# daniabib/ComfyUI_ProPainter_Nodes

Measured on NVIDIA H100. Metric: inpainted frames/sec at 640x360, 80-frame subvideo, higher is better.
Workload: dtype f16

## Files before the change

### comfyui_propainter_nodes_b200/csrc/attention_tc.cu

```cuda
#include "attention.cuh"
#include "wgmma_ops.cuh"

namespace {

constexpr int D = 128, BQ = 128, BKEY = 64, NT = 256, WIN_TOK = 45, RING = 193;
constexpr uint32_t QPANEL = BQ * 128;
constexpr uint32_t KPANEL = BKEY * 128;
constexpr uint32_t QTILE = 2 * QPANEL;
constexpr uint32_t KTILE = 2 * KPANEL;
constexpr uint32_t PTILE = (BKEY / 64) * QPANEL;
constexpr uint32_t SM_Q = 0, SM_K = QTILE, SM_V = SM_K + 2 * KTILE, SM_P = SM_V + 2 * KTILE, SM_END = SM_P + PTILE;

__device__ __forceinline__ uint32_t tile_off(uint32_t panel, int row, int chunk) {
  return (uint32_t)(chunk >> 3) * panel + (uint32_t)row * 128 + (uint32_t)(((chunk & 7) ^ (row & 7)) << 4);
}

__global__ void attn_key_table(int* __restrict__ tab, const int* __restrict__ ring_idx, int nk_max, int kpf, int ntok,
                               int n_pool, int qkv_cs, int pool_cs, int parity) {
  const int win = blockIdx.x;
  const int* ring = ring_idx + win * RING;
  for (int j = threadIdx.x; j < nk_max; j += blockDim.x) {
    const int fi = j / kpf, w = j - fi * kpf;
    const int fr = parity + 2 * fi;
    unsigned e;
    if (w < RING) e = (unsigned)(((long long)fr * ntok + ring[w]) * qkv_cs / 8);
    else e = 0x80000000u | (unsigned)(((long long)fr * n_pool + (w - RING)) * pool_cs / 8);
    tab[(long long)win * nk_max + j] = (int)e;
  }
}

__global__ void __launch_bounds__(NT, 2) window_attention_tc(const PPAttnParams p) {
  using namespace ppx;
  extern __shared__ __align__(1024) uint8_t smem[];
  const uint32_t sbase = smem_u32(smem);

  const int win = blockIdx.y >> 2, head = blockIdx.y & 3, sw = blockIdx.z;
  if (p.win_flags[sw * p.n_win + win] == 0) return;
  const int t = p.sw_t[sw];
  const int frame_base = p.sw_frame_off[sw];
  const int nq = t * WIN_TOK;
  const int q0 = blockIdx.x * BQ;
  if (q0 >= nq) return;
  const int n_tind = (t - p.parity + 1) / 2;
  const int kpf = RING + p.n_pool;
  const int nk = n_tind * kpf;
  const int ntiles = (nk + BKEY - 1) / BKEY;
  const int tid = threadIdx.x;
  const int* ring = p.ring_idx + win * RING;
  const long long ntok = (long long)p.nh * p.nw;

  for (int i = tid; i < BQ * 16; i += NT) {
    const int r = i >> 4, ch = i & 15;
    const int qi = min(q0 + r, nq - 1);
    const int fr = frame_base + qi / WIN_TOK, pos = qi % WIN_TOK;
    const __half* src = p.q + ((long long)fr * ntok + ring[pos]) * p.qkv_cs + head * D + ch * 8;
    cp_async16(sbase + SM_Q + tile_off(QPANEL, r, ch), src, 16);
  }
  const int r0 = tid >> 4, ch = tid & 15;
  const long long fb = frame_base;
  const __half* kb = p.k + fb * ntok * p.qkv_cs + head * D + ch * 8;
  const __half* vb = p.v + fb * ntok * p.qkv_cs + head * D + ch * 8;
  const __half* pkb = p.pk + fb * p.n_pool * p.pool_cs + head * D + ch * 8;
  const __half* pvb = p.pv + fb * p.n_pool * p.pool_cs + head * D + ch * 8;
  const int* ktab = p.key_tab + (long long)win * p.key_tab_stride;
  const uint32_t kv_dst0 = sbase + tile_off(KPANEL, r0, ch);
  auto load_kv = [&](int tile, int stage) {
    const uint32_t dk = kv_dst0 + SM_K + stage * KTILE, dv = kv_dst0 + SM_V + stage * KTILE;
#pragma unroll
    for (int it = 0; it < BKEY / 16; ++it) {
      const int j = tile * BKEY + r0 + 16 * it;
      const __half* ks = kb; const __half* vs = vb;
      uint32_t nbytes = 0;
      if (j < nk) {
        nbytes = 16;
        const int e = __ldg(ktab + j);
        const long long off = (long long)(e & 0x7fffffff) * 8;
        ks = (e < 0 ? pkb : kb) + off;
        vs = (e < 0 ? pvb : vb) + off;
      }
      cp_async16(dk + it * 2048, ks, nbytes);
      cp_async16(dv + it * 2048, vs, nbytes);
    }
    cp_async_commit();
  };
  load_kv(0, 0);

  const int wg = tid >> 7, lane = tid & 31;
  const int rw = 16 * ((tid >> 5) & 3) + (lane >> 2), quad = lane & 3;
  const uint32_t q_rows = (uint32_t)wg * 64 * 128;
  float o[64];
  float m_used[2] = {0.f, 0.f}, m_run[2] = {-1e30f, -1e30f}, row_sum[2] = {0.f, 0.f};
#pragma unroll
  for (int i = 0; i < 64; ++i) o[i] = 0.f;
  for (int j = 0; j < ntiles; ++j) {
    const int stage = j & 1;
    cp_async_wait<0>();
    fence_proxy_async();
    __syncthreads();
    if (j + 1 < ntiles) load_kv(j + 1, stage ^ 1);
    float s[32];
    wgmma_fence();
#pragma unroll
    for (int ks = 0; ks < 8; ++ks) {
      const uint32_t sub = (uint32_t)(ks & 3) * 32;
      wgmma_f16<BKEY>(s, gmma_desc_sw128_kmajor(sbase + SM_Q + (uint32_t)(ks >> 2) * QPANEL + q_rows + sub),
                      gmma_desc_sw128_kmajor(sbase + SM_K + stage * KTILE + (uint32_t)(ks >> 2) * KPANEL + sub), ks != 0 ? 1u : 0u);
    }
    wgmma_commit();
    wgmma_wait<0>();
    wgmma_fence_acc(s);

    const int kvalid = min(BKEY, nk - j * BKEY);
    float mx[2] = {-1e30f, -1e30f};
#pragma unroll
    for (int i = 0; i < 32; ++i) {
      if (8 * (i >> 2) + 2 * quad + (i & 1) >= kvalid) s[i] = -1e30f;
      mx[(i >> 1) & 1] = fmaxf(mx[(i >> 1) & 1], s[i]);
    }
    float f[2];
#pragma unroll
    for (int h = 0; h < 2; ++h) {
      mx[h] = fmaxf(mx[h], __shfl_xor_sync(0xffffffffu, mx[h], 1));
      mx[h] = fmaxf(mx[h], __shfl_xor_sync(0xffffffffu, mx[h], 2));
      const float m_tile = __half2float(__float2half_rn(fmaxf(mx[h] * p.scale_log2, -60000.f)));
      const float m_new = fmaxf(m_run[h], m_tile);
      f[h] = 1.f;
      if (j == 0) m_used[h] = m_new;
      else if (m_new > m_used[h] + 8.f) {
        f[h] = exp2f(m_used[h] - m_new);
        m_used[h] = m_new;
        row_sum[h] *= f[h];
      }
      m_run[h] = m_new;
    }
    if (f[0] != 1.f || f[1] != 1.f) {
#pragma unroll
      for (int i = 0; i < 64; ++i) o[i] *= f[(i >> 1) & 1];
    }
#pragma unroll
    for (int i = 0; i < 32; i += 2) {
      const int h = (i >> 1) & 1;
      const float a = exp2f(fmaf(s[i], p.scale_log2, -m_used[h]));
      const float b = exp2f(fmaf(s[i + 1], p.scale_log2, -m_used[h]));
      row_sum[h] += a + b;
      const int row = wg * 64 + rw + 8 * h;
      *reinterpret_cast<__half2*>(smem + SM_P + tile_off(QPANEL, row, i >> 2) + 4 * quad) = __floats2half2_rn(a, b);
    }
    fence_proxy_async();
    named_bar(1 + wg, 128);
    wgmma_fence();
#pragma unroll
    for (int ks = 0; ks < BKEY / 16; ++ks) {
      const uint64_t adesc = gmma_desc_sw128_kmajor(sbase + SM_P + q_rows + (uint32_t)ks * 32);
      const uint64_t bdesc = gmma_desc_sw128_mnmajor(sbase + SM_V + stage * KTILE + (uint32_t)ks * 2048, KPANEL);
      wgmma_f16<D, 1>(o, adesc, bdesc, 1u);
    }
    wgmma_commit();
    wgmma_wait<0>();
    wgmma_fence_acc(o);
  }

#pragma unroll
  for (int h = 0; h < 2; ++h) {
    row_sum[h] += __shfl_xor_sync(0xffffffffu, row_sum[h], 1);
    row_sum[h] += __shfl_xor_sync(0xffffffffu, row_sum[h], 2);
    const float inv = 1.f / row_sum[h];
    const int qi = q0 + wg * 64 + rw + 8 * h;
    if (qi >= nq) continue;
    const int fr = frame_base + qi / WIN_TOK, pos = qi % WIN_TOK;
    const int tok = ring[pos];
    const int ty = tok / p.nw, tx = tok - ty * p.nw;
    if (ty >= p.gh || tx >= p.gw) continue;
    __half* dst = p.out + (((long long)fr * p.gh + ty) * p.gw + tx) * p.out_cs + head * D + 2 * quad;
#pragma unroll
    for (int g = 0; g < D / 8; ++g)
      *reinterpret_cast<__half2*>(dst + 8 * g) = __floats2half2_rn(o[4 * g + 2 * h] * inv, o[4 * g + 2 * h + 1] * inv);
  }
}

}

int pp_launch_attention_tc(const PPAttnParams& p, int n_sliding, int t_max, cudaStream_t st) {
  const size_t smem = SM_END;
  static bool attr_set = false;
  if (!attr_set) {
    PP_CUDA_CHECK(cudaFuncSetAttribute(window_attention_tc, cudaFuncAttributeMaxDynamicSharedMemorySize, (int)smem));
    PP_CUDA_CHECK(cudaFuncSetAttribute(window_attention_tc, cudaFuncAttributePreferredSharedMemoryCarveout, 100));
    attr_set = true;
  }
  {
    const int kpf = RING + p.n_pool, nk_max = ((t_max - p.parity + 1) / 2) * kpf;
    PP_REQUIRE(p.key_tab != nullptr && p.key_tab_stride >= nk_max, "attention: key table scratch too small (%d < %d)",
               p.key_tab_stride, nk_max);
    attn_key_table<<<p.n_win, 256, 0, st>>>(const_cast<int*>(p.key_tab), p.ring_idx, p.key_tab_stride, kpf, p.nh * p.nw, p.n_pool,
                                           p.qkv_cs, p.pool_cs, p.parity);
    PP_CUDA_CHECK(cudaGetLastError());
  }
  dim3 grid(pp_ceil_div(t_max * WIN_TOK, BQ), p.n_win * 4, n_sliding);
  window_attention_tc<<<grid, NT, smem, st>>>(p);
  PP_CUDA_CHECK(cudaGetLastError());
  return PP_OK;
}
```

### comfyui_propainter_nodes_b200/csrc/wgmma_ops.cuh

```cuda
#pragma once
#include <stdint.h>

namespace ppx {

template <int N, int TB>
struct WgmmaF16;

template <int TB>
struct WgmmaF16<16, TB> {
  static __device__ __forceinline__ void run(float (&d)[8], uint64_t a, uint64_t b, uint32_t acc) {
    asm volatile(
        "{\n.reg .pred p;\nsetp.ne.b32 p, %10, 0;\n"
        "wgmma.mma_async.sync.aligned.m64n16k16.f32.f16.f16 {%0, %1, %2, %3, %4, %5, %6, %7}, %8, %9, p, 1, 1, 0, %11;\n}\n"
        : "+f"(d[0]), "+f"(d[1]), "+f"(d[2]), "+f"(d[3]), "+f"(d[4]), "+f"(d[5]), "+f"(d[6]), "+f"(d[7])
        : "l"(a), "l"(b), "r"(acc), "n"(TB)
        : "memory");
  }
};

template <int TB>
struct WgmmaF16<32, TB> {
  static __device__ __forceinline__ void run(float (&d)[16], uint64_t a, uint64_t b, uint32_t acc) {
    asm volatile(
        "{\n.reg .pred p;\nsetp.ne.b32 p, %18, 0;\n"
// ... 97 lines not shown
        : "+f"(d[0]), "+f"(d[1]), "+f"(d[2]), "+f"(d[3]), "+f"(d[4]), "+f"(d[5]), "+f"(d[6]), "+f"(d[7]), "+f"(d[8]), "+f"(d[9]), "+f"(d[10]), "+f"(d[11]), "+f"(d[12]), "+f"(d[13]), "+f"(d[14]), "+f"(d[15]), "+f"(d[16]), "+f"(d[17]), "+f"(d[18]), "+f"(d[19]), "+f"(d[20]), "+f"(d[21]), "+f"(d[22]), "+f"(d[23]), "+f"(d[24]), "+f"(d[25]), "+f"(d[26]), "+f"(d[27]), "+f"(d[28]), "+f"(d[29]), "+f"(d[30]), "+f"(d[31]), "+f"(d[32]), "+f"(d[33]), "+f"(d[34]), "+f"(d[35]), "+f"(d[36]), "+f"(d[37]), "+f"(d[38]), "+f"(d[39]), "+f"(d[40]), "+f"(d[41]), "+f"(d[42]), "+f"(d[43]), "+f"(d[44]), "+f"(d[45]), "+f"(d[46]), "+f"(d[47]), "+f"(d[48]), "+f"(d[49]), "+f"(d[50]), "+f"(d[51]), "+f"(d[52]), "+f"(d[53]), "+f"(d[54]), "+f"(d[55]), "+f"(d[56]), "+f"(d[57]), "+f"(d[58]), "+f"(d[59]), "+f"(d[60]), "+f"(d[61]), "+f"(d[62]), "+f"(d[63]), "+f"(d[64]), "+f"(d[65]), "+f"(d[66]), "+f"(d[67]), "+f"(d[68]), "+f"(d[69]), "+f"(d[70]), "+f"(d[71]), "+f"(d[72]), "+f"(d[73]), "+f"(d[74]), "+f"(d[75]), "+f"(d[76]), "+f"(d[77]), "+f"(d[78]), "+f"(d[79])
        : "l"(a), "l"(b), "r"(acc), "n"(TB)
        : "memory");
  }
};

template <int TB>
struct WgmmaF16<176, TB> {
  static __device__ __forceinline__ void run(float (&d)[88], uint64_t a, uint64_t b, uint32_t acc) {
    asm volatile(
        "{\n.reg .pred p;\nsetp.ne.b32 p, %90, 0;\n"
        "wgmma.mma_async.sync.aligned.m64n176k16.f32.f16.f16 {%0, %1, %2, %3, %4, %5, %6, %7, %8, %9, %10, %11, %12, %13, %14, %15, %16, %17, %18, %19, %20, %21, %22, %23, %24, %25, %26, %27, %28, %29, %30, %31, %32, %33, %34, %35, %36, %37, %38, %39, %40, %41, %42, %43, %44, %45, %46, %47, %48, %49, %50, %51, %52, %53, %54, %55, %56, %57, %58, %59, %60, %61, %62, %63, %64, %65, %66, %67, %68, %69, %70, %71, %72, %73, %74, %75, %76, %77, %78, %79, %80, %81, %82, %83, %84, %85, %86, %87}, %88, %89, p, 1, 1, 0, %91;\n}\n"
        : "+f"(d[0]), "+f"(d[1]), "+f"(d[2]), "+f"(d[3]), "+f"(d[4]), "+f"(d[5]), "+f"(d[6]), "+f"(d[7]), "+f"(d[8]), "+f"(d[9]), "+f"(d[10]), "+f"(d[11]), "+f"(d[12]), "+f"(d[13]), "+f"(d[14]), "+f"(d[15]), "+f"(d[16]), "+f"(d[17]), "+f"(d[18]), "+f"(d[19]), "+f"(d[20]), "+f"(d[21]), "+f"(d[22]), "+f"(d[23]), "+f"(d[24]), "+f"(d[25]), "+f"(d[26]), "+f"(d[27]), "+f"(d[28]), "+f"(d[29]), "+f"(d[30]), "+f"(d[31]), "+f"(d[32]), "+f"(d[33]), "+f"(d[34]), "+f"(d[35]), "+f"(d[36]), "+f"(d[37]), "+f"(d[38]), "+f"(d[39]), "+f"(d[40]), "+f"(d[41]), "+f"(d[42]), "+f"(d[43]), "+f"(d[44]), "+f"(d[45]), "+f"(d[46]), "+f"(d[47]), "+f"(d[48]), "+f"(d[49]), "+f"(d[50]), "+f"(d[51]), "+f"(d[52]), "+f"(d[53]), "+f"(d[54]), "+f"(d[55]), "+f"(d[56]), "+f"(d[57]), "+f"(d[58]), "+f"(d[59]), "+f"(d[60]), "+f"(d[61]), "+f"(d[62]), "+f"(d[63]), "+f"(d[64]), "+f"(d[65]), "+f"(d[66]), "+f"(d[67]), "+f"(d[68]), "+f"(d[69]), "+f"(d[70]), "+f"(d[71]), "+f"(d[72]), "+f"(d[73]), "+f"(d[74]), "+f"(d[75]), "+f"(d[76]), "+f"(d[77]), "+f"(d[78]), "+f"(d[79]), "+f"(d[80]), "+f"(d[81]), "+f"(d[82]), "+f"(d[83]), "+f"(d[84]), "+f"(d[85]), "+f"(d[86]), "+f"(d[87])
        : "l"(a), "l"(b), "r"(acc), "n"(TB)
        : "memory");
  }
};

template <int TB>
struct WgmmaF16<192, TB> {
  static __device__ __forceinline__ void run(float (&d)[96], uint64_t a, uint64_t b, uint32_t acc) {
    asm volatile(
        "{\n.reg .pred p;\nsetp.ne.b32 p, %98, 0;\n"
        "wgmma.mma_async.sync.aligned.m64n192k16.f32.f16.f16 {%0, %1, %2, %3, %4, %5, %6, %7, %8, %9, %10, %11, %12, %13, %14, %15, %16, %17, %18, %19, %20, %21, %22, %23, %24, %25, %26, %27, %28, %29, %30, %31, %32, %33, %34, %35, %36, %37, %38, %39, %40, %41, %42, %43, %44, %45, %46, %47, %48, %49, %50, %51, %52, %53, %54, %55, %56, %57, %58, %59, %60, %61, %62, %63, %64, %65, %66, %67, %68, %69, %70, %71, %72, %73, %74, %75, %76, %77, %78, %79, %80, %81, %82, %83, %84, %85, %86, %87, %88, %89, %90, %91, %92, %93, %94, %95}, %96, %97, p, 1, 1, 0, %99;\n}\n"
        : "+f"(d[0]), "+f"(d[1]), "+f"(d[2]), "+f"(d[3]), "+f"(d[4]), "+f"(d[5]), "+f"(d[6]), "+f"(d[7]), "+f"(d[8]), "+f"(d[9]), "+f"(d[10]), "+f"(d[11]), "+f"(d[12]), "+f"(d[13]), "+f"(d[14]), "+f"(d[15]), "+f"(d[16]), "+f"(d[17]), "+f"(d[18]), "+f"(d[19]), "+f"(d[20]), "+f"(d[21]), "+f"(d[22]), "+f"(d[23]), "+f"(d[24]), "+f"(d[25]), "+f"(d[26]), "+f"(d[27]), "+f"(d[28]), "+f"(d[29]), "+f"(d[30]), "+f"(d[31]), "+f"(d[32]), "+f"(d[33]), "+f"(d[34]), "+f"(d[35]), "+f"(d[36]), "+f"(d[37]), "+f"(d[38]), "+f"(d[39]), "+f"(d[40]), "+f"(d[41]), "+f"(d[42]), "+f"(d[43]), "+f"(d[44]), "+f"(d[45]), "+f"(d[46]), "+f"(d[47]), "+f"(d[48]), "+f"(d[49]), "+f"(d[50]), "+f"(d[51]), "+f"(d[52]), "+f"(d[53]), "+f"(d[54]), "+f"(d[55]), "+f"(d[56]), "+f"(d[57]), "+f"(d[58]), "+f"(d[59]), "+f"(d[60]), "+f"(d[61]), "+f"(d[62]), "+f"(d[63]), "+f"(d[64]), "+f"(d[65]), "+f"(d[66]), "+f"(d[67]), "+f"(d[68]), "+f"(d[69]), "+f"(d[70]), "+f"(d[71]), "+f"(d[72]), "+f"(d[73]), "+f"(d[74]), "+f"(d[75]), "+f"(d[76]), "+f"(d[77]), "+f"(d[78]), "+f"(d[79]), "+f"(d[80]), "+f"(d[81]), "+f"(d[82]), "+f"(d[83]), "+f"(d[84]), "+f"(d[85]), "+f"(d[86]), "+f"(d[87]), "+f"(d[88]), "+f"(d[89]), "+f"(d[90]), "+f"(d[91]), "+f"(d[92]), "+f"(d[93]), "+f"(d[94]), "+f"(d[95])
        : "l"(a), "l"(b), "r"(acc), "n"(TB)
        : "memory");
  }
};

template <int TB>
struct WgmmaF16<208, TB> {
  static __device__ __forceinline__ void run(float (&d)[104], uint64_t a, uint64_t b, uint32_t acc) {
    asm volatile(
        "{\n.reg .pred p;\nsetp.ne.b32 p, %106, 0;\n"
        "wgmma.mma_async.sync.aligned.m64n208k16.f32.f16.f16 {%0, %1, %2, %3, %4, %5, %6, %7, %8, %9, %10, %11, %12, %13, %14, %15, %16, %17, %18, %19, %20, %21, %22, %23, %24, %25, %26, %27, %28, %29, %30, %31, %32, %33, %34, %35, %36, %37, %38, %39, %40, %41, %42, %43, %44, %45, %46, %47, %48, %49, %50, %51, %52, %53, %54, %55, %56, %57, %58, %59, %60, %61, %62, %63, %64, %65, %66, %67, %68, %69, %70, %71, %72, %73, %74, %75, %76, %77, %78, %79, %80, %81, %82, %83, %84, %85, %86, %87, %88, %89, %90, %91, %92, %93, %94, %95, %96, %97, %98, %99, %100, %101, %102, %103}, %104, %105, p, 1, 1, 0, %107;\n}\n"
        : "+f"(d[0]), "+f"(d[1]), "+f"(d[2]), "+f"(d[3]), "+f"(d[4]), "+f"(d[5]), "+f"(d[6]), "+f"(d[7]), "+f"(d[8]), "+f"(d[9]), "+f"(d[10]), "+f"(d[11]), "+f"(d[12]), "+f"(d[13]), "+f"(d[14]), "+f"(d[15]), "+f"(d[16]), "+f"(d[17]), "+f"(d[18]), "+f"(d[19]), "+f"(d[20]), "+f"(d[21]), "+f"(d[22]), "+f"(d[23]), "+f"(d[24]), "+f"(d[25]), "+f"(d[26]), "+f"(d[27]), "+f"(d[28]), "+f"(d[29]), "+f"(d[30]), "+f"(d[31]), "+f"(d[32]), "+f"(d[33]), "+f"(d[34]), "+f"(d[35]), "+f"(d[36]), "+f"(d[37]), "+f"(d[38]), "+f"(d[39]), "+f"(d[40]), "+f"(d[41]), "+f"(d[42]), "+f"(d[43]), "+f"(d[44]), "+f"(d[45]), "+f"(d[46]), "+f"(d[47]), "+f"(d[48]), "+f"(d[49]), "+f"(d[50]), "+f"(d[51]), "+f"(d[52]), "+f"(d[53]), "+f"(d[54]), "+f"(d[55]), "+f"(d[56]), "+f"(d[57]), "+f"(d[58]), "+f"(d[59]), "+f"(d[60]), "+f"(d[61]), "+f"(d[62]), "+f"(d[63]), "+f"(d[64]), "+f"(d[65]), "+f"(d[66]), "+f"(d[67]), "+f"(d[68]), "+f"(d[69]), "+f"(d[70]), "+f"(d[71]), "+f"(d[72]), "+f"(d[73]), "+f"(d[74]), "+f"(d[75]), "+f"(d[76]), "+f"(d[77]), "+f"(d[78]), "+f"(d[79]), "+f"(d[80]), "+f"(d[81]), "+f"(d[82]), "+f"(d[83]), "+f"(d[84]), "+f"(d[85]), "+f"(d[86]), "+f"(d[87]), "+f"(d[88]), "+f"(d[89]), "+f"(d[90]), "+f"(d[91]), "+f"(d[92]), "+f"(d[93]), "+f"(d[94]), "+f"(d[95]), "+f"(d[96]), "+f"(d[97]), "+f"(d[98]), "+f"(d[99]), "+f"(d[100]), "+f"(d[101]), "+f"(d[102]), "+f"(d[103])
        : "l"(a), "l"(b), "r"(acc), "n"(TB)
        : "memory");
  }
};

template <int TB>
struct WgmmaF16<224, TB> {
  static __device__ __forceinline__ void run(float (&d)[112], uint64_t a, uint64_t b, uint32_t acc) {
    asm volatile(
        "{\n.reg .pred p;\nsetp.ne.b32 p, %114, 0;\n"
        "wgmma.mma_async.sync.aligned.m64n224k16.f32.f16.f16 {%0, %1, %2, %3, %4, %5, %6, %7, %8, %9, %10, %11, %12, %13, %14, %15, %16, %17, %18, %19, %20, %21, %22, %23, %24, %25, %26, %27, %28, %29, %30, %31, %32, %33, %34, %35, %36, %37, %38, %39, %40, %41, %42, %43, %44, %45, %46, %47, %48, %49, %50, %51, %52, %53, %54, %55, %56, %57, %58, %59, %60, %61, %62, %63, %64, %65, %66, %67, %68, %69, %70, %71, %72, %73, %74, %75, %76, %77, %78, %79, %80, %81, %82, %83, %84, %85, %86, %87, %88, %89, %90, %91, %92, %93, %94, %95, %96, %97, %98, %99, %100, %101, %102, %103, %104, %105, %106, %107, %108, %109, %110, %111}, %112, %113, p, 1, 1, 0, %115;\n}\n"
        : "+f"(d[0]), "+f"(d[1]), "+f"(d[2]), "+f"(d[3]), "+f"(d[4]), "+f"(d[5]), "+f"(d[6]), "+f"(d[7]), "+f"(d[8]), "+f"(d[9]), "+f"(d[10]), "+f"(d[11]), "+f"(d[12]), "+f"(d[13]), "+f"(d[14]), "+f"(d[15]), "+f"(d[16]), "+f"(d[17]), "+f"(d[18]), "+f"(d[19]), "+f"(d[20]), "+f"(d[21]), "+f"(d[22]), "+f"(d[23]), "+f"(d[24]), "+f"(d[25]), "+f"(d[26]), "+f"(d[27]), "+f"(d[28]), "+f"(d[29]), "+f"(d[30]), "+f"(d[31]), "+f"(d[32]), "+f"(d[33]), "+f"(d[34]), "+f"(d[35]), "+f"(d[36]), "+f"(d[37]), "+f"(d[38]), "+f"(d[39]), "+f"(d[40]), "+f"(d[41]), "+f"(d[42]), "+f"(d[43]), "+f"(d[44]), "+f"(d[45]), "+f"(d[46]), "+f"(d[47]), "+f"(d[48]), "+f"(d[49]), "+f"(d[50]), "+f"(d[51]), "+f"(d[52]), "+f"(d[53]), "+f"(d[54]), "+f"(d[55]), "+f"(d[56]), "+f"(d[57]), "+f"(d[58]), "+f"(d[59]), "+f"(d[60]), "+f"(d[61]), "+f"(d[62]), "+f"(d[63]), "+f"(d[64]), "+f"(d[65]), "+f"(d[66]), "+f"(d[67]), "+f"(d[68]), "+f"(d[69]), "+f"(d[70]), "+f"(d[71]), "+f"(d[72]), "+f"(d[73]), "+f"(d[74]), "+f"(d[75]), "+f"(d[76]), "+f"(d[77]), "+f"(d[78]), "+f"(d[79]), "+f"(d[80]), "+f"(d[81]), "+f"(d[82]), "+f"(d[83]), "+f"(d[84]), "+f"(d[85]), "+f"(d[86]), "+f"(d[87]), "+f"(d[88]), "+f"(d[89]), "+f"(d[90]), "+f"(d[91]), "+f"(d[92]), "+f"(d[93]), "+f"(d[94]), "+f"(d[95]), "+f"(d[96]), "+f"(d[97]), "+f"(d[98]), "+f"(d[99]), "+f"(d[100]), "+f"(d[101]), "+f"(d[102]), "+f"(d[103]), "+f"(d[104]), "+f"(d[105]), "+f"(d[106]), "+f"(d[107]), "+f"(d[108]), "+f"(d[109]), "+f"(d[110]), "+f"(d[111])
        : "l"(a), "l"(b), "r"(acc), "n"(TB)
        : "memory");
  }
};

template <int TB>
struct WgmmaF16<240, TB> {
  static __device__ __forceinline__ void run(float (&d)[120], uint64_t a, uint64_t b, uint32_t acc) {
    asm volatile(
        "{\n.reg .pred p;\nsetp.ne.b32 p, %122, 0;\n"
        "wgmma.mma_async.sync.aligned.m64n240k16.f32.f16.f16 {%0, %1, %2, %3, %4, %5, %6, %7, %8, %9, %10, %11, %12, %13, %14, %15, %16, %17, %18, %19, %20, %21, %22, %23, %24, %25, %26, %27, %28, %29, %30, %31, %32, %33, %34, %35, %36, %37, %38, %39, %40, %41, %42, %43, %44, %45, %46, %47, %48, %49, %50, %51, %52, %53, %54, %55, %56, %57, %58, %59, %60, %61, %62, %63, %64, %65, %66, %67, %68, %69, %70, %71, %72, %73, %74, %75, %76, %77, %78, %79, %80, %81, %82, %83, %84, %85, %86, %87, %88, %89, %90, %91, %92, %93, %94, %95, %96, %97, %98, %99, %100, %101, %102, %103, %104, %105, %106, %107, %108, %109, %110, %111, %112, %113, %114, %115, %116, %117, %118, %119}, %120, %121, p, 1, 1, 0, %123;\n}\n"
        : "+f"(d[0]), "+f"(d[1]), "+f"(d[2]), "+f"(d[3]), "+f"(d[4]), "+f"(d[5]), "+f"(d[6]), "+f"(d[7]), "+f"(d[8]), "+f"(d[9]), "+f"(d[10]), "+f"(d[11]), "+f"(d[12]), "+f"(d[13]), "+f"(d[14]), "+f"(d[15]), "+f"(d[16]), "+f"(d[17]), "+f"(d[18]), "+f"(d[19]), "+f"(d[20]), "+f"(d[21]), "+f"(d[22]), "+f"(d[23]), "+f"(d[24]), "+f"(d[25]), "+f"(d[26]), "+f"(d[27]), "+f"(d[28]), "+f"(d[29]), "+f"(d[30]), "+f"(d[31]), "+f"(d[32]), "+f"(d[33]), "+f"(d[34]), "+f"(d[35]), "+f"(d[36]), "+f"(d[37]), "+f"(d[38]), "+f"(d[39]), "+f"(d[40]), "+f"(d[41]), "+f"(d[42]), "+f"(d[43]), "+f"(d[44]), "+f"(d[45]), "+f"(d[46]), "+f"(d[47]), "+f"(d[48]), "+f"(d[49]), "+f"(d[50]), "+f"(d[51]), "+f"(d[52]), "+f"(d[53]), "+f"(d[54]), "+f"(d[55]), "+f"(d[56]), "+f"(d[57]), "+f"(d[58]), "+f"(d[59]), "+f"(d[60]), "+f"(d[61]), "+f"(d[62]), "+f"(d[63]), "+f"(d[64]), "+f"(d[65]), "+f"(d[66]), "+f"(d[67]), "+f"(d[68]), "+f"(d[69]), "+f"(d[70]), "+f"(d[71]), "+f"(d[72]), "+f"(d[73]), "+f"(d[74]), "+f"(d[75]), "+f"(d[76]), "+f"(d[77]), "+f"(d[78]), "+f"(d[79]), "+f"(d[80]), "+f"(d[81]), "+f"(d[82]), "+f"(d[83]), "+f"(d[84]), "+f"(d[85]), "+f"(d[86]), "+f"(d[87]), "+f"(d[88]), "+f"(d[89]), "+f"(d[90]), "+f"(d[91]), "+f"(d[92]), "+f"(d[93]), "+f"(d[94]), "+f"(d[95]), "+f"(d[96]), "+f"(d[97]), "+f"(d[98]), "+f"(d[99]), "+f"(d[100]), "+f"(d[101]), "+f"(d[102]), "+f"(d[103]), "+f"(d[104]), "+f"(d[105]), "+f"(d[106]), "+f"(d[107]), "+f"(d[108]), "+f"(d[109]), "+f"(d[110]), "+f"(d[111]), "+f"(d[112]), "+f"(d[113]), "+f"(d[114]), "+f"(d[115]), "+f"(d[116]), "+f"(d[117]), "+f"(d[118]), "+f"(d[119])
        : "l"(a), "l"(b), "r"(acc), "n"(TB)
        : "memory");
  }
};

template <int TB>
struct WgmmaF16<256, TB> {
  static __device__ __forceinline__ void run(float (&d)[128], uint64_t a, uint64_t b, uint32_t acc) {
    asm volatile(
        "{\n.reg .pred p;\nsetp.ne.b32 p, %130, 0;\n"
        "wgmma.mma_async.sync.aligned.m64n256k16.f32.f16.f16 {%0, %1, %2, %3, %4, %5, %6, %7, %8, %9, %10, %11, %12, %13, %14, %15, %16, %17, %18, %19, %20, %21, %22, %23, %24, %25, %26, %27, %28, %29, %30, %31, %32, %33, %34, %35, %36, %37, %38, %39, %40, %41, %42, %43, %44, %45, %46, %47, %48, %49, %50, %51, %52, %53, %54, %55, %56, %57, %58, %59, %60, %61, %62, %63, %64, %65, %66, %67, %68, %69, %70, %71, %72, %73, %74, %75, %76, %77, %78, %79, %80, %81, %82, %83, %84, %85, %86, %87, %88, %89, %90, %91, %92, %93, %94, %95, %96, %97, %98, %99, %100, %101, %102, %103, %104, %105, %106, %107, %108, %109, %110, %111, %112, %113, %114, %115, %116, %117, %118, %119, %120, %121, %122, %123, %124, %125, %126, %127}, %128, %129, p, 1, 1, 0, %131;\n}\n"
        : "+f"(d[0]), "+f"(d[1]), "+f"(d[2]), "+f"(d[3]), "+f"(d[4]), "+f"(d[5]), "+f"(d[6]), "+f"(d[7]), "+f"(d[8]), "+f"(d[9]), "+f"(d[10]), "+f"(d[11]), "+f"(d[12]), "+f"(d[13]), "+f"(d[14]), "+f"(d[15]), "+f"(d[16]), "+f"(d[17]), "+f"(d[18]), "+f"(d[19]), "+f"(d[20]), "+f"(d[21]), "+f"(d[22]), "+f"(d[23]), "+f"(d[24]), "+f"(d[25]), "+f"(d[26]), "+f"(d[27]), "+f"(d[28]), "+f"(d[29]), "+f"(d[30]), "+f"(d[31]), "+f"(d[32]), "+f"(d[33]), "+f"(d[34]), "+f"(d[35]), "+f"(d[36]), "+f"(d[37]), "+f"(d[38]), "+f"(d[39]), "+f"(d[40]), "+f"(d[41]), "+f"(d[42]), "+f"(d[43]), "+f"(d[44]), "+f"(d[45]), "+f"(d[46]), "+f"(d[47]), "+f"(d[48]), "+f"(d[49]), "+f"(d[50]), "+f"(d[51]), "+f"(d[52]), "+f"(d[53]), "+f"(d[54]), "+f"(d[55]), "+f"(d[56]), "+f"(d[57]), "+f"(d[58]), "+f"(d[59]), "+f"(d[60]), "+f"(d[61]), "+f"(d[62]), "+f"(d[63]), "+f"(d[64]), "+f"(d[65]), "+f"(d[66]), "+f"(d[67]), "+f"(d[68]), "+f"(d[69]), "+f"(d[70]), "+f"(d[71]), "+f"(d[72]), "+f"(d[73]), "+f"(d[74]), "+f"(d[75]), "+f"(d[76]), "+f"(d[77]), "+f"(d[78]), "+f"(d[79]), "+f"(d[80]), "+f"(d[81]), "+f"(d[82]), "+f"(d[83]), "+f"(d[84]), "+f"(d[85]), "+f"(d[86]), "+f"(d[87]), "+f"(d[88]), "+f"(d[89]), "+f"(d[90]), "+f"(d[91]), "+f"(d[92]), "+f"(d[93]), "+f"(d[94]), "+f"(d[95]), "+f"(d[96]), "+f"(d[97]), "+f"(d[98]), "+f"(d[99]), "+f"(d[100]), "+f"(d[101]), "+f"(d[102]), "+f"(d[103]), "+f"(d[104]), "+f"(d[105]), "+f"(d[106]), "+f"(d[107]), "+f"(d[108]), "+f"(d[109]), "+f"(d[110]), "+f"(d[111]), "+f"(d[112]), "+f"(d[113]), "+f"(d[114]), "+f"(d[115]), "+f"(d[116]), "+f"(d[117]), "+f"(d[118]), "+f"(d[119]), "+f"(d[120]), "+f"(d[121]), "+f"(d[122]), "+f"(d[123]), "+f"(d[124]), "+f"(d[125]), "+f"(d[126]), "+f"(d[127])
        : "l"(a), "l"(b), "r"(acc), "n"(TB)
        : "memory");
  }
};

template <int N, int TRANS_B = 0>
__device__ __forceinline__ void wgmma_f16(float (&d)[N / 2], uint64_t a, uint64_t b, uint32_t accumulate) {
  WgmmaF16<N, TRANS_B>::run(d, a, b, accumulate);
}

template <int N>
struct WgmmaTF32;

template <>
struct WgmmaTF32<16> {
  static __device__ __forceinline__ void run(float (&d)[8], uint64_t a, uint64_t b, uint32_t acc) {
    asm volatile(
        "{\n.reg .pred p;\nsetp.ne.b32 p, %10, 0;\n"
        "wgmma.mma_async.sync.aligned.m64n16k8.f32.tf32.tf32 {%0, %1, %2, %3, %4, %5, %6, %7}, %8, %9, p, 1, 1;\n}\n"
        : "+f"(d[0]), "+f"(d[1]), "+f"(d[2]), "+f"(d[3]), "+f"(d[4]), "+f"(d[5]), "+f"(d[6]), "+f"(d[7])
        : "l"(a), "l"(b), "r"(acc)
        : "memory");
  }
};

template <>
struct WgmmaTF32<32> {
  static __device__ __forceinline__ void run(float (&d)[16], uint64_t a, uint64_t b, uint32_t acc) {
    asm volatile(
        "{\n.reg .pred p;\nsetp.ne.b32 p, %18, 0;\n"
        "wgmma.mma_async.sync.aligned.m64n32k8.f32.tf32.tf32 {%0, %1, %2, %3, %4, %5, %6, %7, %8, %9, %10, %11, %12, %13, %14, %15}, %16, %17, p, 1, 1;\n}\n"
        : "+f"(d[0]), "+f"(d[1]), "+f"(d[2]), "+f"(d[3]), "+f"(d[4]), "+f"(d[5]), "+f"(d[6]), "+f"(d[7]), "+f"(d[8]), "+f"(d[9]), "+f"(d[10]), "+f"(d[11]), "+f"(d[12]), "+f"(d[13]), "+f"(d[14]), "+f"(d[15])
        : "l"(a), "l"(b), "r"(acc)
        : "memory");
  }
};

template <>
struct WgmmaTF32<48> {
  static __device__ __forceinline__ void run(float (&d)[24], uint64_t a, uint64_t b, uint32_t acc) {
    asm volatile(
        "{\n.reg .pred p;\nsetp.ne.b32 p, %26, 0;\n"
        "wgmma.mma_async.sync.aligned.m64n48k8.f32.tf32.tf32 {%0, %1, %2, %3, %4, %5, %6, %7, %8, %9, %10, %11, %12, %13, %14, %15, %16, %17, %18, %19, %20, %21, %22, %23}, %24, %25, p, 1, 1;\n}\n"
        : "+f"(d[0]), "+f"(d[1]), "+f"(d[2]), "+f"(d[3]), "+f"(d[4]), "+f"(d[5]), "+f"(d[6]), "+f"(d[7]), "+f"(d[8]), "+f"(d[9]), "+f"(d[10]), "+f"(d[11]), "+f"(d[12]), "+f"(d[13]), "+f"(d[14]), "+f"(d[15]), "+f"(d[16]), "+f"(d[17]), "+f"(d[18]), "+f"(d[19]), "+f"(d[20]), "+f"(d[21]), "+f"(d[22]), "+f"(d[23])
        : "l"(a), "l"(b), "r"(acc)
        : "memory");
  }
};

template <>
struct WgmmaTF32<64> {
  static __device__ __forceinline__ void run(float (&d)[32], uint64_t a, uint64_t b, uint32_t acc) {
    asm volatile(
        "{\n.reg .pred p;\nsetp.ne.b32 p, %34, 0;\n"
        "wgmma.mma_async.sync.aligned.m64n64k8.f32.tf32.tf32 {%0, %1, %2, %3, %4, %5, %6, %7, %8, %9, %10, %11, %12, %13, %14, %15, %16, %17, %18, %19, %20, %21, %22, %23, %24, %25, %26, %27, %28, %29, %30, %31}, %32, %33, p, 1, 1;\n}\n"
        : "+f"(d[0]), "+f"(d[1]), "+f"(d[2]), "+f"(d[3]), "+f"(d[4]), "+f"(d[5]), "+f"(d[6]), "+f"(d[7]), "+f"(d[8]), "+f"(d[9]), "+f"(d[10]), "+f"(d[11]), "+f"(d[12]), "+f"(d[13]), "+f"(d[14]), "+f"(d[15]), "+f"(d[16]), "+f"(d[17]), "+f"(d[18]), "+f"(d[19]), "+f"(d[20]), "+f"(d[21]), "+f"(d[22]), "+f"(d[23]), "+f"(d[24]), "+f"(d[25]), "+f"(d[26]), "+f"(d[27]), "+f"(d[28]), "+f"(d[29]), "+f"(d[30]), "+f"(d[31])
        : "l"(a), "l"(b), "r"(acc)
        : "memory");
  }
};

template <>
struct WgmmaTF32<80> {
  static __device__ __forceinline__ void run(float (&d)[40], uint64_t a, uint64_t b, uint32_t acc) {
    asm volatile(
        "{\n.reg .pred p;\nsetp.ne.b32 p, %42, 0;\n"
        "wgmma.mma_async.sync.aligned.m64n80k8.f32.tf32.tf32 {%0, %1, %2, %3, %4, %5, %6, %7, %8, %9, %10, %11, %12, %13, %14, %15, %16, %17, %18, %19, %20, %21, %22, %23, %24, %25, %26, %27, %28, %29, %30, %31, %32, %33, %34, %35, %36, %37, %38, %39}, %40, %41, p, 1, 1;\n}\n"
        : "+f"(d[0]), "+f"(d[1]), "+f"(d[2]), "+f"(d[3]), "+f"(d[4]), "+f"(d[5]), "+f"(d[6]), "+f"(d[7]), "+f"(d[8]), "+f"(d[9]), "+f"(d[10]), "+f"(d[11]), "+f"(d[12]), "+f"(d[13]), "+f"(d[14]), "+f"(d[15]), "+f"(d[16]), "+f"(d[17]), "+f"(d[18]), "+f"(d[19]), "+f"(d[20]), "+f"(d[21]), "+f"(d[22]), "+f"(d[23]), "+f"(d[24]), "+f"(d[25]), "+f"(d[26]), "+f"(d[27]), "+f"(d[28]), "+f"(d[29]), "+f"(d[30]), "+f"(d[31]), "+f"(d[32]), "+f"(d[33]), "+f"(d[34]), "+f"(d[35]), "+f"(d[36]), "+f"(d[37]), "+f"(d[38]), "+f"(d[39])
        : "l"(a), "l"(b), "r"(acc)
        : "memory");
  }
};

template <>
struct WgmmaTF32<96> {
  static __device__ __forceinline__ void run(float (&d)[48], uint64_t a, uint64_t b, uint32_t acc) {
    asm volatile(
        "{\n.reg .pred p;\nsetp.ne.b32 p, %50, 0;\n"
        "wgmma.mma_async.sync.aligned.m64n96k8.f32.tf32.tf32 {%0, %1, %2, %3, %4, %5, %6, %7, %8, %9, %10, %11, %12, %13, %14, %15, %16, %17, %18, %19, %20, %21, %22, %23, %24, %25, %26, %27, %28, %29, %30, %31, %32, %33, %34, %35, %36, %37, %38, %39, %40, %41, %42, %43, %44, %45, %46, %47}, %48, %49, p, 1, 1;\n}\n"
        : "+f"(d[0]), "+f"(d[1]), "+f"(d[2]), "+f"(d[3]), "+f"(d[4]), "+f"(d[5]), "+f"(d[6]), "+f"(d[7]), "+f"(d[8]), "+f"(d[9]), "+f"(d[10]), "+f"(d[11]), "+f"(d[12]), "+f"(d[13]), "+f"(d[14]), "+f"(d[15]), "+f"(d[16]), "+f"(d[17]), "+f"(d[18]), "+f"(d[19]), "+f"(d[20]), "+f"(d[21]), "+f"(d[22]), "+f"(d[23]), "+f"(d[24]), "+f"(d[25]), "+f"(d[26]), "+f"(d[27]), "+f"(d[28]), "+f"(d[29]), "+f"(d[30]), "+f"(d[31]), "+f"(d[32]), "+f"(d[33]), "+f"(d[34]), "+f"(d[35]), "+f"(d[36]), "+f"(d[37]), "+f"(d[38]), "+f"(d[39]), "+f"(d[40]), "+f"(d[41]), "+f"(d[42]), "+f"(d[43]), "+f"(d[44]), "+f"(d[45]), "+f"(d[46]), "+f"(d[47])
        : "l"(a), "l"(b), "r"(acc)
        : "memory");
  }
};

template <>
struct WgmmaTF32<112> {
  static __device__ __forceinline__ void run(float (&d)[56], uint64_t a, uint64_t b, uint32_t acc) {
    asm volatile(
        "{\n.reg .pred p;\nsetp.ne.b32 p, %58, 0;\n"
        "wgmma.mma_async.sync.aligned.m64n112k8.f32.tf32.tf32 {%0, %1, %2, %3, %4, %5, %6, %7, %8, %9, %10, %11, %12, %13, %14, %15, %16, %17, %18, %19, %20, %21, %22, %23, %24, %25, %26, %27, %28, %29, %30, %31, %32, %33, %34, %35, %36, %37, %38, %39, %40, %41, %42, %43, %44, %45, %46, %47, %48, %49, %50, %51, %52, %53, %54, %55}, %56, %57, p, 1, 1;\n}\n"
        : "+f"(d[0]), "+f"(d[1]), "+f"(d[2]), "+f"(d[3]), "+f"(d[4]), "+f"(d[5]), "+f"(d[6]), "+f"(d[7]), "+f"(d[8]), "+f"(d[9]), "+f"(d[10]), "+f"(d[11]), "+f"(d[12]), "+f"(d[13]), "+f"(d[14]), "+f"(d[15]), "+f"(d[16]), "+f"(d[17]), "+f"(d[18]), "+f"(d[19]), "+f"(d[20]), "+f"(d[21]), "+f"(d[22]), "+f"(d[23]), "+f"(d[24]), "+f"(d[25]), "+f"(d[26]), "+f"(d[27]), "+f"(d[28]), "+f"(d[29]), "+f"(d[30]), "+f"(d[31]), "+f"(d[32]), "+f"(d[33]), "+f"(d[34]), "+f"(d[35]), "+f"(d[36]), "+f"(d[37]), "+f"(d[38]), "+f"(d[39]), "+f"(d[40]), "+f"(d[41]), "+f"(d[42]), "+f"(d[43]), "+f"(d[44]), "+f"(d[45]), "+f"(d[46]), "+f"(d[47]), "+f"(d[48]), "+f"(d[49]), "+f"(d[50]), "+f"(d[51]), "+f"(d[52]), "+f"(d[53]), "+f"(d[54]), "+f"(d[55])
        : "l"(a), "l"(b), "r"(acc)
// ... 119 lines not shown
```

Baseline: 182.0.

## Warp-specialize window attention with mbarrier KV pipeline and register-operand PV wgmma

Splits the attention block into a producer warpgroup that streams K/V tiles via cp.async into a 5-stage ring guarded by full/empty mbarriers, and two consumer warpgroups that own the math. Consumers issue the next QK^T wgmma before the softmax of the current tile and keep P in registers, feeding the PV wgmma through a new register-A variant instead of shared memory. This removes block-wide syncs and the P smem round trip. In exchange occupancy drops to one block per SM, register counts are redistributed with setmaxnreg, and more shared memory is used.

```diff
diff --git a/comfyui_propainter_nodes_b200/csrc/attention_tc.cu b/comfyui_propainter_nodes_b200/csrc/attention_tc.cu
--- a/comfyui_propainter_nodes_b200/csrc/attention_tc.cu
+++ b/comfyui_propainter_nodes_b200/csrc/attention_tc.cu
@@ -3,13 +3,14 @@
 
 namespace {
 
-constexpr int D = 128, BQ = 128, BKEY = 64, NT = 256, WIN_TOK = 45, RING = 193;
+constexpr int D = 128, BQ = 128, BKEY = 64, WIN_TOK = 45, RING = 193, STAGES = 5;
+constexpr int NUM_CONSUMERS = 256, NT = NUM_CONSUMERS + 128;
 constexpr uint32_t QPANEL = BQ * 128;
 constexpr uint32_t KPANEL = BKEY * 128;
 constexpr uint32_t QTILE = 2 * QPANEL;
 constexpr uint32_t KTILE = 2 * KPANEL;
-constexpr uint32_t PTILE = (BKEY / 64) * QPANEL;
-constexpr uint32_t SM_Q = 0, SM_K = QTILE, SM_V = SM_K + 2 * KTILE, SM_P = SM_V + 2 * KTILE, SM_END = SM_P + PTILE;
+constexpr uint32_t STAGE = 2 * KTILE;
+constexpr uint32_t SM_Q = 0, SM_KV = QTILE, SM_BAR = SM_KV + STAGES * STAGE, SM_END = SM_BAR + 2 * STAGES * 8;
 
 __device__ __forceinline__ uint32_t tile_off(uint32_t panel, int row, int chunk) {
   return (uint32_t)(chunk >> 3) * panel + (uint32_t)row * 128 + (uint32_t)(((chunk & 7) ^ (row & 7)) << 4);
@@ -29,10 +30,12 @@
   }
 }
 
-__global__ void __launch_bounds__(NT, 2) window_attention_tc(const PPAttnParams p) {
+__global__ void __launch_bounds__(NT, 1) window_attention_tc(const PPAttnParams p) {
   using namespace ppx;
   extern __shared__ __align__(1024) uint8_t smem[];
   const uint32_t sbase = smem_u32(smem);
+  uint64_t* full = reinterpret_cast<uint64_t*>(smem + SM_BAR);
+  uint64_t* empty = full + STAGES;
 
   const int win = blockIdx.y >> 2, head = blockIdx.y & 3, sw = blockIdx.z;
   if (p.win_flags[sw * p.n_win + win] == 0) return;
@@ -49,66 +52,92 @@
   const int* ring = p.ring_idx + win * RING;
   const long long ntok = (long long)p.nh * p.nw;
 
-  for (int i = tid; i < BQ * 16; i += NT) {
-    const int r = i >> 4, ch = i & 15;
-    const int qi = min(q0 + r, nq - 1);
-    const int fr = frame_base + qi / WIN_TOK, pos = qi % WIN_TOK;
-    const __half* src = p.q + ((long long)fr * ntok + ring[pos]) * p.qkv_cs + head * D + ch * 8;
-    cp_async16(sbase + SM_Q + tile_off(QPANEL, r, ch), src, 16);
-  }
-  const int r0 = tid >> 4, ch = tid & 15;
-  const long long fb = frame_base;
-  const __half* kb = p.k + fb * ntok * p.qkv_cs + head * D + ch * 8;
-  const __half* vb = p.v + fb * ntok * p.qkv_cs + head * D + ch * 8;
-  const __half* pkb = p.pk + fb * p.n_pool * p.pool_cs + head * D + ch * 8;
-  const __half* pvb = p.pv + fb * p.n_pool * p.pool_cs + head * D + ch * 8;
-  const int* ktab = p.key_tab + (long long)win * p.key_tab_stride;
-  const uint32_t kv_dst0 = sbase + tile_off(KPANEL, r0, ch);
-  auto load_kv = [&](int tile, int stage) {
-    const uint32_t dk = kv_dst0 + SM_K + stage * KTILE, dv = kv_dst0 + SM_V + stage * KTILE;
-#pragma unroll
-    for (int it = 0; it < BKEY / 16; ++it) {
-      const int j = tile * BKEY + r0 + 16 * it;
-      const __half* ks = kb; const __half* vs = vb;
-      uint32_t nbytes = 0;
-      if (j < nk) {
-        nbytes = 16;
-        const int e = __ldg(ktab + j);
-        const long long off = (long long)(e & 0x7fffffff) * 8;
-        ks = (e < 0 ? pkb : kb) + off;
-        vs = (e < 0 ? pvb : vb) + off;
+  if (tid == 0) {
+    for (int s = 0; s < STAGES; ++s) {
+      mbar_init(&full[s], 128);
+      mbar_init(&empty[s], NUM_CONSUMERS);
+    }
+    mbar_fence_init();
+  }
+  __syncthreads();
+
+  if (tid >= NUM_CONSUMERS) {
+    setmaxnreg_dec<40>();
+    const int ptid = tid - NUM_CONSUMERS;
+    for (int i = ptid; i < BQ * 16; i += 128) {
+      const int r = i >> 4, ch = i & 15;
+      const int qi = min(q0 + r, nq - 1);
+      const int fr = frame_base + qi / WIN_TOK, pos = qi % WIN_TOK;
+      const __half* src = p.q + ((long long)fr * ntok + ring[pos]) * p.qkv_cs + head * D + ch * 8;
+      cp_async16(sbase + SM_Q + tile_off(QPANEL, r, ch), src, 16);
+    }
+    const int r0 = ptid >> 4, ch = ptid & 15;
+    const long long fb = frame_base;
+    const __half* kb = p.k + fb * ntok * p.qkv_cs + head * D + ch * 8;
+    const __half* vb = p.v + fb * ntok * p.qkv_cs + head * D + ch * 8;
+    const __half* pkb = p.pk + fb * p.n_pool * p.pool_cs + head * D + ch * 8;
+    const __half* pvb = p.pv + fb * p.n_pool * p.pool_cs + head * D + ch * 8;
+    const int* ktab = p.key_tab + (long long)win * p.key_tab_stride;
+    const uint32_t kv_dst0 = sbase + SM_KV + tile_off(KPANEL, r0, ch);
+    for (int j = 0; j < ntiles; ++j) {
+      const int s = j % STAGES;
+      mbar_wait(&empty[s], ((j / STAGES) & 1) ^ 1);
+      const uint32_t dk = kv_dst0 + s * STAGE, dv = dk + KTILE;
+#pragma unroll
+      for (int it = 0; it < BKEY / 8; ++it) {
+        const int key = j * BKEY + r0 + 8 * it;
+        const __half* ks = kb; const __half* vs = vb;
+        uint32_t nbytes = 0;
+        if (key < nk) {
+          nbytes = 16;
+          const int e = __ldg(ktab + key);
+          const long long off = (long long)(e & 0x7fffffff) * 8;
+          ks = (e < 0 ? pkb : kb) + off;
+          vs = (e < 0 ? pvb : vb) + off;
+        }
+        cp_async16(dk + it * 1024, ks, nbytes);
+        cp_async16(dv + it * 1024, vs, nbytes);
       }
-      cp_async16(dk + it * 2048, ks, nbytes);
-      cp_async16(dv + it * 2048, vs, nbytes);
+      cp_async_arrive_noinc(&full[s]);
     }
     cp_async_commit();
-  };
-  load_kv(0, 0);
-
+    cp_async_wait<0>();
+    return;
+  }
+
+  setmaxnreg_inc<232>();
   const int wg = tid >> 7, lane = tid & 31;
   const int rw = 16 * ((tid >> 5) & 3) + (lane >> 2), quad = lane & 3;
   const uint32_t q_rows = (uint32_t)wg * 64 * 128;
-  float o[64];
+  float o[64], sa[32], sb[32];
   float m_used[2] = {0.f, 0.f}, m_run[2] = {-1e30f, -1e30f}, row_sum[2] = {0.f, 0.f};
 #pragma unroll
   for (int i = 0; i < 64; ++i) o[i] = 0.f;
-  for (int j = 0; j < ntiles; ++j) {
-    const int stage = j & 1;
-    cp_async_wait<0>();
+  wgmma_fence_acc(o);
+
+  auto issue_s = [&](int j, float (&s)[32]) {
+    const int st = j % STAGES;
+    mbar_wait(&full[st], (uint32_t)(j / STAGES) & 1u);
     fence_proxy_async();
-    __syncthreads();
-    if (j + 1 < ntiles) load_kv(j + 1, stage ^ 1);
-    float s[32];
     wgmma_fence();
 #pragma unroll
     for (int ks = 0; ks < 8; ++ks) {
       const uint32_t sub = (uint32_t)(ks & 3) * 32;
       wgmma_f16<BKEY>(s, gmma_desc_sw128_kmajor(sbase + SM_Q + (uint32_t)(ks >> 2) * QPANEL + q_rows + sub),
-                      gmma_desc_sw128_kmajor(sbase + SM_K + stage * KTILE + (uint32_t)(ks >> 2) * KPANEL + sub), ks != 0 ? 1u : 0u);
+                      gmma_desc_sw128_kmajor(sbase + SM_KV + st * STAGE + (uint32_t)(ks >> 2) * KPANEL + sub), ks != 0 ? 1u : 0u);
     }
     wgmma_commit();
-    wgmma_wait<0>();
+  };
+  auto step = [&](int j, float (&s)[32], float (&s_next)[32], bool has_next) {
+    if (has_next) {
+      issue_s(j + 1, s_next);
+      wgmma_wait<1>();
+    } else {
+      wgmma_wait<0>();
+    }
     wgmma_fence_acc(s);
+    wgmma_fence_acc(o);
+    if (j > 0) mbar_arrive(&empty[(j - 1) % STAGES]);
 
     const int kvalid = min(BKEY, nk - j * BKEY);
     float mx[2] = {-1e30f, -1e30f};
@@ -137,28 +166,40 @@
 #pragma unroll
       for (int i = 0; i < 64; ++i) o[i] *= f[(i >> 1) & 1];
     }
+    uint32_t pa[16];
 #pragma unroll
     for (int i = 0; i < 32; i += 2) {
       const int h = (i >> 1) & 1;
       const float a = exp2f(fmaf(s[i], p.scale_log2, -m_used[h]));
       const float b = exp2f(fmaf(s[i + 1], p.scale_log2, -m_used[h]));
       row_sum[h] += a + b;
-      const int row = wg * 64 + rw + 8 * h;
-      *reinterpret_cast<__half2*>(smem + SM_P + tile_off(QPANEL, row, i >> 2) + 4 * quad) = __floats2half2_rn(a, b);
-    }
-    fence_proxy_async();
-    named_bar(1 + wg, 128);
+      const __half2 ab = __floats2half2_rn(a, b);
+      pa[i >> 1] = *reinterpret_cast<const uint32_t*>(&ab);
+    }
     wgmma_fence();
+    const int st = j % STAGES;
 #pragma unroll
     for (int ks = 0; ks < BKEY / 16; ++ks) {
-      const uint64_t adesc = gmma_desc_sw128_kmajor(sbase + SM_P + q_rows + (uint32_t)ks * 32);
-      const uint64_t bdesc = gmma_desc_sw128_mnmajor(sbase + SM_V + stage * KTILE + (uint32_t)ks * 2048, KPANEL);
-      wgmma_f16<D, 1>(o, adesc, bdesc, 1u);
+      const uint64_t bdesc = gmma_desc_sw128_mnmajor(sbase + SM_KV + st * STAGE + KTILE + (uint32_t)ks * 2048, KPANEL);
+      wgmma_f16_rs<D, 1>(o, *reinterpret_cast<const uint32_t(*)[4]>(pa + 4 * ks), bdesc, 1u);
     }
     wgmma_commit();
-    wgmma_wait<0>();
-    wgmma_fence_acc(o);
-  }
+  };
+
+  issue_s(0, sa);
+  int j = 0;
+  for (; j + 2 < ntiles; j += 2) {
+    step(j, sa, sb, true);
+    step(j + 1, sb, sa, true);
+  }
+  if (j + 1 < ntiles) {
+    step(j, sa, sb, true);
+    step(j + 1, sb, sa, false);
+  } else {
+    step(j, sa, sb, false);
+  }
+  wgmma_wait<0>();
+  wgmma_fence_acc(o);
 
 #pragma unroll
   for (int h = 0; h < 2; ++h) {
diff --git a/comfyui_propainter_nodes_b200/csrc/wgmma_ops.cuh b/comfyui_propainter_nodes_b200/csrc/wgmma_ops.cuh
--- a/comfyui_propainter_nodes_b200/csrc/wgmma_ops.cuh
+++ b/comfyui_propainter_nodes_b200/csrc/wgmma_ops.cuh
@@ -203,6 +203,26 @@
   WgmmaF16<N, TRANS_B>::run(d, a, b, accumulate);
 }
 
+template <int N, int TB>
+struct WgmmaF16RS;
+
+template <int TB>
+struct WgmmaF16RS<128, TB> {
+  static __device__ __forceinline__ void run(float (&d)[64], const uint32_t (&a)[4], uint64_t b, uint32_t acc) {
+    asm volatile(
+        "{\n.reg .pred p;\nsetp.ne.b32 p, %69, 0;\n"
+        "wgmma.mma_async.sync.aligned.m64n128k16.f32.f16.f16 {%0, %1, %2, %3, %4, %5, %6, %7, %8, %9, %10, %11, %12, %13, %14, %15, %16, %17, %18, %19, %20, %21, %22, %23, %24, %25, %26, %27, %28, %29, %30, %31, %32, %33, %34, %35, %36, %37, %38, %39, %40, %41, %42, %43, %44, %45, %46, %47, %48, %49, %50, %51, %52, %53, %54, %55, %56, %57, %58, %59, %60, %61, %62, %63}, {%64, %65, %66, %67}, %68, p, 1, 1, %70;\n}\n"
+        : "+f"(d[0]), "+f"(d[1]), "+f"(d[2]), "+f"(d[3]), "+f"(d[4]), "+f"(d[5]), "+f"(d[6]), "+f"(d[7]), "+f"(d[8]), "+f"(d[9]), "+f"(d[10]), "+f"(d[11]), "+f"(d[12]), "+f"(d[13]), "+f"(d[14]), "+f"(d[15]), "+f"(d[16]), "+f"(d[17]), "+f"(d[18]), "+f"(d[19]), "+f"(d[20]), "+f"(d[21]), "+f"(d[22]), "+f"(d[23]), "+f"(d[24]), "+f"(d[25]), "+f"(d[26]), "+f"(d[27]), "+f"(d[28]), "+f"(d[29]), "+f"(d[30]), "+f"(d[31]), "+f"(d[32]), "+f"(d[33]), "+f"(d[34]), "+f"(d[35]), "+f"(d[36]), "+f"(d[37]), "+f"(d[38]), "+f"(d[39]), "+f"(d[40]), "+f"(d[41]), "+f"(d[42]), "+f"(d[43]), "+f"(d[44]), "+f"(d[45]), "+f"(d[46]), "+f"(d[47]), "+f"(d[48]), "+f"(d[49]), "+f"(d[50]), "+f"(d[51]), "+f"(d[52]), "+f"(d[53]), "+f"(d[54]), "+f"(d[55]), "+f"(d[56]), "+f"(d[57]), "+f"(d[58]), "+f"(d[59]), "+f"(d[60]), "+f"(d[61]), "+f"(d[62]), "+f"(d[63])
+        : "r"(a[0]), "r"(a[1]), "r"(a[2]), "r"(a[3]), "l"(b), "r"(acc), "n"(TB)
+        : "memory");
+  }
+};
+
+template <int N, int TRANS_B = 0>
+__device__ __forceinline__ void wgmma_f16_rs(float (&d)[N / 2], const uint32_t (&a)[4], uint64_t b, uint32_t accumulate) {
+  WgmmaF16RS<N, TRANS_B>::run(d, a, b, accumulate);
+}
+
 template <int N>
 struct WgmmaTF32;
 
```

Result: no change. 182.9, median of 6 (+0.5%).
